# quocdat32461997/ggpm

Measured on AMD Instinct MI355X. Metric: HierMPNEncoder fwd+bwd target row (SURVEY 8(d): encoder + KL heads + optimizer, tree fixed-point hint on; full depth loops in full_depth_loops, the full VAE fwd+bwd row in vae_step) of BASELINE's molecules/sec VAE fwd+bwd (hidden=300, depth=20, batch=32), higher is better.
Workload: dtype f32

## Files before the change

### ggpm_amd/csrc/common.h

```cpp
#pragma once
#include <hip/hip_runtime.h>
#include <stdint.h>
#include <stdlib.h>
#include <atomic>
#include <mutex>
#include "../../include/ggpm_hip.h"

typedef float f32x4 __attribute__((ext_vector_type(4)));
typedef float f32x16 __attribute__((ext_vector_type(16)));

#define GGPM_WAVE 64

#define GGPM_CHECK_LAUNCH()                                   \
    do {                                                      \
        if (hipGetLastError() != hipSuccess) return GGPM_ERR_LAUNCH; \
    } while (0)

#define GGPM_CLEAR_STALE_ERROR() (void)hipGetLastError()

#ifdef GGPM_DEV_SWITCHES
inline const char* ggpm_dev_env(const char* name) { return getenv(name); }
#else
inline const char* ggpm_dev_env(const char*) { return nullptr; }
#endif
// ... 92 lines not shown
    static const ggpm_level_opts none = {};
    return opts ? *opts : none;
}
int ggpm_gru_bias_u_grad(int E1, int H, int depth, int lo, float* work, float* dbu, float* csws, const ggpm_level_opts* opts,
                         ggpm_stream_t stream);
int ggpm_gru_sparse_weight_grads(int E1, int H, int depth, const float* Hs, const float* Ss, const float* Gs, float* work,
                                 size_t work_bytes, float* dWz_h, int ld_dwz, float* dUr, int ld_dur, float* dbu, float* dWh_h,
                                 int ld_dwh, const ggpm_level_opts* opts, ggpm_stream_t stream);
int ggpm_lstm_sparse_weight_grads(int E1, int H, int depth, const float* Hs, const float* Ss, float* work, size_t work_bytes,
                                  float* dWi_h, int ld_dwi, float* dWo_h, int ld_dwo, float* dWu_h, int ld_dwu, float* dWf_h,
                                  int ld_dwf, const ggpm_level_opts* opts, ggpm_stream_t stream);
hipEvent_t ggpm_wgrad_event(int i);

bool ggpm_bf16_storage_applies(int E1, int H);
int ggpm_sum_slots_any(const float* src, int slots, size_t slot_floats, float* out, bool src_bf16, ggpm_stream_t stream);
int ggpm_colsum_any(const float* A, int lda, int rows, int cols, float* out, float* scratch, bool a_bf16, ggpm_stream_t stream);

void ggpm_timing_tag(int tag);
void ggpm_timing_begin(int which, hipStream_t s, double flops);
void ggpm_timing_end(int which, hipStream_t s);
```

### ggpm_amd/csrc/encoder.hip

```cpp
#include "common.h"
#include <condition_variable>
#include <cstring>
#include <cstdlib>
#include <deque>
#include <functional>
#include <mutex>
#include <thread>

hipEvent_t ggpm_wgrad_event(int i);

namespace {

struct Arena {
    char* base;
    size_t off;
    bool overflow;
    size_t cap;
    template <typename T>
    T* take(size_t n) {
        const size_t bytes = (n * sizeof(T) + 255) & ~(size_t)255;
        T* p = base ? reinterpret_cast<T*>(base + off) : nullptr;
        off += bytes;
        if (base && off > cap) overflow = true;
        return p;
// ... 271 lines not shown

inline bool bf16_stored(const Dims& d, int E1) { return d.gate_dtype == 1 && ggpm_bf16_storage_applies(E1, d.H); }
inline int run_steps(const Dims& d, int level, int depth, int E1) {
    static const bool off = ggpm_dev_env("GGPM_TREE_FIXED_POINT") && atoi(ggpm_dev_env("GGPM_TREE_FIXED_POINT")) == 0;
    if (off || level == 2 || bf16_stored(d, E1) || d.tree_chain <= 0 || d.tree_chain + 1 >= depth) return depth;
    return d.tree_chain + 1;
}

inline int backward_lo(const Dims& d, int level, int depth, int E1) {
    static const bool off = ggpm_dev_env("GGPM_TREE_FIXED_POINT") && atoi(ggpm_dev_env("GGPM_TREE_FIXED_POINT")) == 0;
    if (off || level == 2 || bf16_stored(d, E1) || d.tree_chain <= 0) return 1;
    const int lo = depth - d.tree_chain + 1;
    return lo < 1 ? 1 : lo;
}

int replicate_tail(const Dims& d, int E1, int depth, int run, int level, const LevelSaved& L, ggpm_stream_t s) {
    if (run >= depth) return GGPM_OK;
    const size_t slot = (size_t)E1 * d.Hp, ds = (size_t)depth * slot;
    const int blo = backward_lo(d, level, depth, E1);
    ReplicateArgs r = {};
    int n = 0;
    auto add = [&](float* base, int src, int lo, int hi) {
        r.base[n] = base; r.src[n] = src; r.lo[n] = lo > src ? lo : src + 1; r.hi[n] = hi; ++n;
    };
    add(L.Hs, run, blo, depth);
    if (L.Cs) add(L.Cs, run, blo, depth);
    add(L.Qs, run, blo, depth - 1);
    for (int k = 0; k < 5; ++k) add(L.St + k * ds, run - 1, blo - 1, depth - 1);
    r.slot4 = slot / 4;
    dim3 grid((unsigned)ggpm_ceil_div((int)r.slot4, 256 * 4), n);
    replicate_slots_k<<<grid, 256, 0, (hipStream_t)s>>>(r);
    return GGPM_OK;
}

int level_forward(const Dims& d, int E1, int N1, int I, int depth, const float* x, int ldx, float* const* P, int level,
                  const Csr& pred, const Csr& agr, LevelSaved& L, ggpm_stream_t s) {
    const int H = d.H, Hp = d.Hp;
    const size_t slot = (size_t)E1 * Hp;
    const int run = run_steps(d, level, depth, E1);
    struct Tag { Tag(int level) { ggpm_timing_tag(3 - level); } ~Tag() { ggpm_timing_tag(0); } } tag(level);
    ggpm_level_opts o = level_opts(d);
    o.run_depth = run;
    const bool infer = L.hout != nullptr;
    o.h_out = L.hout;
    const float* result = infer ? L.hout : L.Hs + (size_t)depth * slot;
    if (d.lstm) {
        const float* W[4] = {P[lq(level, Q_WI)], P[lq(level, Q_WOG)], P[lq(level, Q_WU)], P[lq(level, Q_WF)]};
        const float* b[4] = {P[lq(level, Q_BI)], P[lq(level, Q_BOG)], P[lq(level, Q_BU)], P[lq(level, Q_BF)]};
        GgpmGemmProblem gp[4];
        for (int k = 0; k < 4; ++k) gp[k] = {x, ldx, W[k], I + H, L.X + k * slot, Hp, Hp, b[k], 0, GGPM_ACT_NONE, 0};
        CK(ggpm_gemm_grouped(0, 1, E1, H, I, 4, gp, s));
        const size_t dsl = (size_t)depth * slot;
        CK(ggpm_lstm_forward(E1, H, depth, L.X, L.X + slot, L.X + 2 * slot, L.X + 3 * slot, W[0] + I, I + H, W[1] + I, I + H,
                             W[2] + I, I + H, W[3] + I, I + H, pred.rowptr, pred.col, L.Hs, L.Cs, L.Qs,
                             infer ? nullptr : L.St, infer ? nullptr : L.St + dsl, infer ? nullptr : L.St + 2 * dsl,
                             infer ? nullptr : L.St + 3 * dsl, infer ? nullptr : L.St + 4 * dsl, L.wpack, infer ? 0 : 1, &o, s));
        if (!infer) CK(replicate_tail(d, E1, depth, run, level, L, s));
        CK(ggpm_segment_sum(result, Hp, agr.rowptr, agr.col, N1, H, L.nei, Hp, 0, Hp, s));
        return GGPM_OK;
    }
// ... 272 lines not shown
        return GGPM_OK;
    });
}

int level_backward(const Dims& d, int E1, int I, int depth, const float* x, int ldx, float* const* P, float* const* G,
                   int level, const Csr& pred, const LevelSaved& L, const float* dHD, float* dX, float* level_work,
                   float* dx, int lddx, BwdWork& w, Streams& st) {
    const int H = d.H, Hp = d.Hp;
    const size_t slot = (size_t)E1 * Hp, ds = (size_t)depth * slot;
    const int blo = backward_lo(d, level, depth, E1);
    struct Tag { Tag(int level) { ggpm_timing_tag(3 - level); } ~Tag() { ggpm_timing_tag(0); } } tag(level);
    static const bool xsum_env = !(ggpm_dev_env("GGPM_SKIP_XSUM") && atoi(ggpm_dev_env("GGPM_SKIP_XSUM")) == 0);
    const bool skip_xsum = xsum_env && dx == nullptr && depth > 1;
    ggpm_level_opts o = level_opts(d);
    o.lo = blo;
    o.skip_x_sums = skip_xsum;
    if (d.lstm) {
        const float* W[4] = {P[lq(level, Q_WI)], P[lq(level, Q_WOG)], P[lq(level, Q_WU)], P[lq(level, Q_WF)]};
        float* dW[4] = {G[lq(level, Q_WI)], G[lq(level, Q_WOG)], G[lq(level, Q_WU)], G[lq(level, Q_WF)]};
        float* db[4] = {G[lq(level, Q_BI)], G[lq(level, Q_BOG)], G[lq(level, Q_BU)], G[lq(level, Q_BF)]};
        CK(ggpm_lstm_backward(E1, H, depth, L.X + 3 * slot, W[0] + I, I + H, W[1] + I, I + H, W[2] + I, I + H, W[3] + I, I + H,
                              pred.rowptr, pred.col, pred.rowptrT, pred.colT, L.Hs, L.Cs, L.Qs, L.St, L.St + ds,
                              L.St + 2 * ds, L.St + 3 * ds, L.St + 4 * ds, dHD, dX, dX + slot, dX + 2 * slot, dX + 3 * slot,
                              dW[0] + I, I + H, dW[1] + I, I + H, dW[2] + I, I + H, dW[3] + I, I + H, level_work,
                              w.level_work_bytes, 0, &o, st.main));
        if (dx) {
            const float* A[4] = {dX, dX + slot, dX + 2 * slot, dX + 3 * slot};
            const int lda[4] = {Hp, Hp, Hp, Hp}, ldb[4] = {I + H, I + H, I + H, I + H}, K[4] = {H, H, H, H};
            CK(ggpm_gemm_ksegments(0, E1, I, 4, A, lda, W, ldb, K, dx, lddx, lddx, nullptr, 0, GGPM_ACT_NONE, 0, st.main));
        }
// ... 254 lines not shown
```

### ggpm_amd/csrc/gemm.hip

```cpp
#include <stdio.h>
#include <stdlib.h>
#include "common.h"

namespace {

constexpr int BM = 64, BN = 64, BK = 32, LDT = 68;

struct GemmArgs {
    int M, N, K;
    const float* A; int lda;
    const float* B; int ldb;
    float* C; int ldc; int n_pad;
    const float* bias;
    int accumulate, act, zero_row0;
    int vecA, vecB;
    int k_chunk;
    float* ws;
    unsigned long long* dbg;
    int nseg;
    const float* segA[GGPM_GEMM_MAX_GROUP];
    const float* segB[GGPM_GEMM_MAX_GROUP];
    int seg_lda[GGPM_GEMM_MAX_GROUP], seg_ldb[GGPM_GEMM_MAX_GROUP], segK[GGPM_GEMM_MAX_GROUP];
};

// ... 1203 lines not shown
        gg.p[i].k_chunk = ggpm_round_up(ggpm_ceil_div(K[i], splits), (bf16 || split) ? BTK : TK);
        gg.p[i].ws = ws + (size_t)i * splits * slabs_per_chunk * (slab / sizeof(float));
    }
    for (int i = count; i < GGPM_GEMM_MAX_GROUP; ++i) gg.p[i] = gg.p[0];
    hipStream_t s = (hipStream_t)stream;
    const int tiles_n = ggpm_ceil_div(N, TN), tiles_m = ggpm_ceil_div(M, TM);
    if (in16) gemm_tn_tall_bf16<true><<<dim3(tiles_n, tiles_m, splits * count), 256, 0, s>>>(gg, splits);
    else if (bf16) gemm_tn_tall_bf16<false><<<dim3(tiles_n, tiles_m, splits * count), 256, 0, s>>>(gg, splits);
    else if (split) launch_tall_split(gg, dim3(tiles_n, tiles_m, splits * count), splits, s);
    else gemm_tn_tall<<<dim3(tiles_n, tiles_m, splits * count), 256, 0, s>>>(gg, splits);
    tall_reduce<<<dim3(tiles_n * tiles_m * 100, count), 256, 0, s>>>(gg, splits * slabs_per_chunk, tiles_n, tiles_n * tiles_m);
    GGPM_CHECK_LAUNCH();
    return GGPM_OK;
}

bool ggpm_bf16_storage_applies(int E1, int H) {
    static const int use_tall = [] { const char* e = ggpm_dev_env("GGPM_GEMM_TALL"); return e ? atoi(e) : 1; }();
    return use_tall && E1 >= 6144 && tall_shape(H, H, E1);
}
extern "C" int ggpm_level_bf16_storage(int E1, int H) { return ggpm_bf16_storage_applies(E1, H) ? 1 : 0; }

extern "C" int ggpm_gemm_tn_bf16_applies(int M, int N, int K) {
    static const int use_tall = [] { const char* e = ggpm_dev_env("GGPM_GEMM_TALL"); return e ? atoi(e) : 1; }();
    return use_tall && M > 0 && N > 0 && K > 0 && tall_shape(M, N, K) ? 1 : 0;
}

extern "C" int ggpm_gemm_tn_bf16(int M, int N, int K, const float* A, int lda, const float* B, int ldb, float* C, int ldc,
                                 float* ws, size_t ws_bytes, ggpm_stream_t stream) {
    if (!A || !B || !C || !ws || M <= 0 || N <= 0 || K <= 0 || ldc < N) return GGPM_ERR_ARG;
    const GgpmGemmProblem p = {A, lda, B, ldb, C, ldc, N, nullptr, 0, GGPM_ACT_NONE, 0};
// ... 184 lines not shown
```

### ggpm_amd/csrc/mpn_gru.hip

```cpp
#include "tile_mma.h"
#include <cstdlib>
#include <cstdio>

__global__ void ggpm_pack_weight_kernel(GgpmPackArgs a) {
    const int Hp = a.Hp, H = a.H, KC = Hp / 16;
    const int lane = threadIdx.x;
    const int kc = blockIdx.x, t = blockIdx.y, m = blockIdx.z;
    const float* __restrict__ W = a.W[m];
    const int ldw = a.ldw[m];
    const int out = 16 * t + (lane & 15);
    if (a.bf16 == 2) {
        const int KC32 = ggpm_kc32_dev(Hp);
        float x[8];
#pragma unroll
        for (int i = 0; i < 8; ++i) {
            const int k = 32 * kc + 8 * (lane >> 4) + i;
            x[i] = (out < H && k < H) ? (a.transpose ? W[(size_t)k * ldw + out] : W[(size_t)out * ldw + k]) : 0.f;
        }
        uint2 lo[3], hi[3];
        ggpm_split3(make_float4(x[0], x[1], x[2], x[3]), lo[0], lo[1], lo[2]);
        ggpm_split3(make_float4(x[4], x[5], x[6], x[7]), hi[0], hi[1], hi[2]);
        __bf16* dst = reinterpret_cast<__bf16*>(a.dst) + (size_t)m * 2 * ggpm_packed_matrix_floats(Hp, 2);
#pragma unroll
        for (int pl = 0; pl < 3; ++pl)
// ... 857 lines not shown
        if (gathered) { a0.src_h = o.gather_h; a0.src_idx = o.gather_idx; }
        const size_t lds_b = bf16 == 2 ? ggpm_split_image_bytes(ROWS, Hp) : (size_t)ROWS * (Hp + 4) * sizeof(float);
        dim3 grid_a(ggpm_ceil_div(E1, ROWS), ggpm_ceil_div(Hp / 16, tg0));
        if (bf16 == 2) { set_lds(gru_fwd_b<2, 1>, lds_b); gru_fwd_b<2, 1><<<grid_a, GGPM_NWA * 64, lds_b, s>>>(a0); }
        else if (bf16 == 1) { set_lds(gru_fwd_b<1, 1>, lds_b); gru_fwd_b<1, 1><<<grid_a, GGPM_NWA * 64, lds_b, s>>>(a0); }
        else { set_lds(gru_fwd_b<0, 1>, lds_b); gru_fwd_b<0, 1><<<grid_a, GGPM_NWA * 64, lds_b, s>>>(a0); }
    }

    const int tg = pick_tg(E1, Hp / 16);
    const double flops1 = 2.0 * (double)(E1 - 1) * H * H;
    static const char* const abl = ggpm_dev_env("GGPM_ABLATE");
    const bool infer = !save_for_backward && o.h_out;
    const bool st16 = bf16 == 1 && !frozen && (save_for_backward || infer) && ggpm_bf16_storage_applies(E1, H);
    int run_depth = o.run_depth;
    if (run_depth <= 0 || run_depth > depth || frozen || !(save_for_backward || infer)) run_depth = depth;
    for (int t = 1; t <= run_depth; ++t) {
        GruFwdArgs a = {};
        a.E1 = E1; a.Hp = Hp; a.tg = tg; a.Xz = Xz; a.Xr = Xr; a.Xh = Xh;
        a.Wz = pWz; a.Wh = pWh; a.Ur = pUr; a.bu = pbu; a.rowptr = pred_rowptr; a.col = pred_col;
        a.ablate = abl ? atoi(abl) : 0;
        a.frozen = frozen;
        a.bf16 = bf16;
        a.st16 = st16 ? 1 : 0;
        a.h0_zero = (t == 1 && !frozen) ? 1 : 0;
        if (save_for_backward) {
            a.Hprev = ggpm_slot_ptr(Hs, t - 1, slot, st16); a.Hnew = ggpm_slot_ptr(Hs, t, slot, st16);
            a.Hout = (st16 && t == depth) ? Hs + (size_t)depth * slot : nullptr;
            a.Qprev = ggpm_slot_ptr(Qs, t - 1, slot, st16);
            a.Qnew = (t < depth) ? ggpm_slot_ptr(Qs, t, slot, st16) : nullptr;
            a.S = ggpm_slot_ptr(Ss, t - 1, slot, st16); a.G = ggpm_slot_ptr(Gs, t - 1, slot, st16);
            a.Z = ggpm_slot_ptr(Zs, t - 1, slot, st16); a.M = ggpm_slot_ptr(Ms, t - 1, slot, st16);
            a.R = Rs + (size_t)(t - 1) * slot;
        } else if (infer) {
            a.Hprev = ggpm_slot_ptr(Hs, (t - 1) & 1, slot, st16); a.Hnew = ggpm_slot_ptr(Hs, t & 1, slot, st16);
            a.Qprev = ggpm_slot_ptr(Qs, (t - 1) & 1, slot, st16); a.Qnew = ggpm_slot_ptr(Qs, t & 1, slot, st16);
            if (t == run_depth) {
                if (st16) a.Hout = o.h_out;
                else a.Hnew = o.h_out;
            }
            a.S = a.G = a.Z = a.M = a.R = nullptr;
        } else {
            a.Hprev = Hs + (size_t)((t - 1) & 1) * slot; a.Hnew = Hs + (size_t)(t & 1) * slot;
            a.Qprev = Qs + (size_t)((t - 1) & 1) * slot; a.Qnew = Qs + (size_t)(t & 1) * slot;
            a.S = a.G = a.Z = a.M = a.R = nullptr;
        }
        launch_fwd(a, rt2, save_for_backward != 0, t < depth, flops1, s);
    }
    GGPM_CHECK_LAUNCH();
    return GGPM_OK;
}

extern "C" int ggpm_gru_forward(int E1, int H, int depth, const float* Xz, const float* Xr, const float* Xh,
                                const float* Wz_h, int ld_wz, const float* Ur, int ld_ur, const float* bu,
                                const float* Wh_h, int ld_wh, const int32_t* pred_rowptr,
                                const int32_t* pred_col, float* Hs, float* Qs, float* Ss, float* Gs, float* Zs,
                                float* Ms, float* Rs, float* wpack, int save_for_backward,
                                const ggpm_level_opts* opts, ggpm_stream_t stream) {
    return gru_forward_impl(E1, H, depth, Xz, Xr, Xh, Wz_h, ld_wz, Ur, ld_ur, bu, Wh_h, ld_wh, pred_rowptr, pred_col,
                            Hs, Qs, Ss, Gs, Zs, Ms, Rs, wpack, save_for_backward, nullptr, nullptr, ggpm_opts_or_default(opts),
                            stream);
}
// ... 82 lines not shown
    }

    {
        GgpmPackArgs pk = {};
        pk.W[0] = Wz_h; pk.ldw[0] = ld_wz; pk.W[1] = Wh_h; pk.ldw[1] = ld_wh; pk.W[2] = Ur; pk.ldw[2] = ld_ur;
        pk.H = H; pk.Hp = Hp; pk.transpose = 1; pk.dst = pWzT; pk.bias = nullptr; pk.bias_out = nullptr; pk.bf16 = bf16;
        if (!o.weights_packed) ggpm_launch_pack(pk, 3, s);
    }
    if (depth == 1 && !frozen) (void)hipMemsetAsync(dXr, 0, slot * sizeof(float), s);

    const int tg = pick_tg(E1, Hp / 16);
    const double flops1 = 2.0 * (double)(E1 - 1) * H * H;
    const bool st16 = bf16 == 1 && !frozen && ggpm_bf16_storage_applies(E1, H);
    int lo = o.lo;
    if (lo < 1 || lo > depth || frozen) lo = 1;
    for (int t = depth; t >= lo; --t) {
        GruBwdArgs a = {};
        a.E1 = E1; a.Hp = Hp; a.tg = tg; a.first = (t == depth);
        a.Xr = Xr;
        a.st16 = st16 ? 1 : 0;
        a.Hcur = ggpm_slot_ptr(Hs, t, slot, st16);
        a.Qcur = (t < depth) ? ggpm_slot_ptr(Qs, t, slot, st16) : nullptr;
        a.S = ggpm_slot_ptr(Ss, t - 1, slot, st16); a.Z = ggpm_slot_ptr(Zs, t - 1, slot, st16);
        a.M = ggpm_slot_ptr(Ms, t - 1, slot, st16);
        a.R = Rs + (size_t)(t - 1) * slot;
        a.dHD = dHD;
        a.dSin = dSb[(t + 1) & 1]; a.dGin = dGb[(t + 1) & 1];
        a.dSout = dSb[t & 1]; a.dGout = dGb[t & 1];
        a.DQ = (t < depth) ? ggpm_slot_ptr(DQ, t, slot, st16) : nullptr;
        a.frozen = frozen; a.carry = carry; a.final_pass = 0; a.dHin = nullptr;
        a.DMP = ggpm_slot_ptr(DMP, t - 1, slot, st16); a.DZP = ggpm_slot_ptr(DZP, t - 1, slot, st16); a.DSD = DSD;
        a.dXz = dXz; a.dXr = dXr; a.dXh = dXh;
        a.WzT = pWzT; a.WhT = pWhT; a.UrT = pUrT; a.bf16 = bf16;
        a.srowptr = succ_rowptr; a.scol = succ_col;
        a.skip_xsum = skip_xsum ? 1 : 0;
        launch_bwd(a, rt2, t > 1 || frozen != nullptr, flops1, s);
    }
    GGPM_CHECK_LAUNCH();

    if (frozen) {
// ... 55 lines not shown
    const int Hp = ggpm_padded_hidden(H);
    hipStream_t s = (hipStream_t)stream;
    const size_t HH = (size_t)Hp * Hp, slot = (size_t)E1 * Hp;
    float* w = work + 3 * ggpm_packed_matrix_slot(Hp);
    float* DMP = w; w += (size_t)depth * slot;
    float* DZP = w; w += (size_t)depth * slot;
    float* DQ = w; w += (size_t)depth * slot;
    w += 6 * slot;
    float* csws = w; w += (size_t)256 * Hp;
    float* skws = w;
    const size_t skbytes = work_bytes - (size_t)((char*)skws - (char*)work);
    const int KD = (depth - lo + 1) * E1;
    const bool st16 = o.gate_dtype == 1 && !with_slot0 && ggpm_bf16_storage_applies(E1, H);
    const int tall_mode = st16 ? 2 : (o.gate_dtype == 1 ? 1 : 0);
    int rc;
    ggpm_gemm_problem gp[3] = {{ggpm_slot_ptr(DMP, lo - 1, slot, st16), Hp, ggpm_slot_ptr(Gs, lo - 1, slot, st16), Hp, dWh_h, ld_dwh, H,
                                nullptr, 0, GGPM_ACT_NONE, 0},
                               {ggpm_slot_ptr(DZP, lo - 1, slot, st16), Hp, ggpm_slot_ptr(Ss, lo - 1, slot, st16), Hp, dWz_h, ld_dwz, H,
                                nullptr, 0, GGPM_ACT_NONE, 0},
                               {nullptr, Hp, nullptr, Hp, dUr, ld_dur, H, nullptr, 0, GGPM_ACT_NONE, 0}};
    int Ks[3] = {KD, KD, 0};
    if (depth > lo || with_slot0) {
        const int first_slot = with_slot0 ? 0 : lo;
        const int KQ = (depth - first_slot) * E1;
        const float* dq0 = ggpm_slot_ptr(DQ, first_slot, slot, st16);
        gp[2].A = dq0;
        gp[2].B = ggpm_slot_ptr(Hs, first_slot, slot, st16);
        Ks[2] = KQ;
        if (!skip_bu) {
            rc = ggpm_colsum_any(dq0, Hp, KQ, H, dbu, csws, st16, stream);
// ... 24 lines not shown
        return GGPM_OK;
    }
    const bool st16 = ggpm_opts_or_default(opts).gate_dtype == 1 && ggpm_bf16_storage_applies(E1, H);
    return ggpm_colsum_any(ggpm_slot_ptr(DQ, lo, slot, st16), Hp, (depth - lo) * E1, H, dbu, csws, st16, stream);
}

namespace {
template <bool B16>
__global__ void __launch_bounds__(256) sum_slots_k(const float* __restrict__ src, int slots, size_t slot4, float* __restrict__ out) {
    const size_t i = (size_t)blockIdx.x * 256 + threadIdx.x;
    if (i >= slot4) return;
    float4 acc = ggpm_ldx<B16>(src, 4 * i);
    for (int t = 1; t < slots; ++t) acc = acc + ggpm_ldx<B16>(src, 4 * ((size_t)t * slot4 + i));
    reinterpret_cast<float4*>(out)[i] = acc;
}
}

extern "C" int ggpm_sum_slots(const float* src, int slots, size_t slot_floats, float* out, ggpm_stream_t stream) {
    return ggpm_sum_slots_any(src, slots, slot_floats, out, false, stream);
}

int ggpm_sum_slots_any(const float* src, int slots, size_t slot_floats, float* out, bool src_bf16, ggpm_stream_t stream) {
    GGPM_CLEAR_STALE_ERROR();
    if (!src || !out || slots <= 0 || slot_floats == 0 || (slot_floats & 3)) return GGPM_ERR_ARG;
    const size_t slot4 = slot_floats / 4;
    if (src_bf16) sum_slots_k<true><<<(unsigned)((slot4 + 255) / 256), 256, 0, (hipStream_t)stream>>>(src, slots, slot4, out);
    else sum_slots_k<false><<<(unsigned)((slot4 + 255) / 256), 256, 0, (hipStream_t)stream>>>(src, slots, slot4, out);
    GGPM_CHECK_LAUNCH();
    return GGPM_OK;
}
// ... 55 lines not shown
```

### ggpm_amd/csrc/mpn_lstm.hip

```cpp
#include "tile_mma.h"
#include <cstdlib>

namespace {

constexpr int ROWS = 16;

struct LstmFwdArgs {
    int E1, Hp, tg;
    const float *Xi, *Xo, *Xu, *Xf;
    const float *Hprev, *Cprev, *Qprev;
    float *Hnew, *Cnew, *Qnew;
    float *S, *I, *O, *U, *F;
    const float *Wi, *Wo, *Wu, *Wf;
    const int32_t *rowptr, *col;
    const unsigned char* frozen;
    int fuse_b;
    int h0_zero;
    int bf16;
    int st16;
    float* Hout;
    const float *src_h, *src_c;
    const int32_t* src_idx;
};

// ... 744 lines not shown
        dim3 grid_a(ggpm_ceil_div(E1, ROWS), ggpm_ceil_div(Hp / 16, tg));
        if (bf16 == 2) { set_lds(lstm_fwd_b<2, 1>, lb); lstm_fwd_b<2, 1><<<grid_a, GGPM_NWA * 64, lb, s>>>(a0); }
        else if (bf16 == 1) { set_lds(lstm_fwd_b<1, 1>, lb); lstm_fwd_b<1, 1><<<grid_a, GGPM_NWA * 64, lb, s>>>(a0); }
        else { set_lds(lstm_fwd_b<0, 1>, lb); lstm_fwd_b<0, 1><<<grid_a, GGPM_NWA * 64, lb, s>>>(a0); }
    } else {
        (void)hipMemsetAsync(Hs, 0, slot * sizeof(float), s);
        (void)hipMemsetAsync(Cs, 0, slot * sizeof(float), s);
        (void)hipMemsetAsync(Qs, 0, slot * sizeof(float), s);
    }

    const double flops1 = 2.0 * (double)(E1 - 1) * H * H;
    const bool infer = !save_for_backward && o.h_out;
    int run_depth = o.run_depth;
    if (run_depth <= 0 || run_depth > depth || frozen || !(save_for_backward || infer)) run_depth = depth;
    const bool st16 = bf16 == 1 && !frozen && (save_for_backward || infer) && ggpm_bf16_storage_applies(E1, H);
    for (int t = 1; t <= run_depth; ++t) {
        LstmFwdArgs a = {};
        a.E1 = E1; a.Hp = Hp; a.tg = tg; a.Xi = Xi; a.Xo = Xo; a.Xu = Xu; a.Xf = Xf;
        a.Wi = pWi; a.Wo = pWo; a.Wu = pWu; a.Wf = pWf; a.rowptr = pred_rowptr; a.col = pred_col;
        a.frozen = frozen;
        a.bf16 = bf16;
        a.st16 = st16 ? 1 : 0;
        a.h0_zero = (t == 1 && !frozen) ? 1 : 0;
        if (save_for_backward) {
            a.Hprev = ggpm_slot_ptr(Hs, t - 1, slot, st16); a.Hnew = ggpm_slot_ptr(Hs, t, slot, st16);
            a.Hout = (st16 && t == depth) ? Hs + (size_t)depth * slot : nullptr;
            a.Cprev = Cs + (size_t)(t - 1) * slot; a.Cnew = Cs + (size_t)t * slot;
            a.Qprev = ggpm_slot_ptr(Qs, t - 1, slot, st16); a.Qnew = (t < depth) ? ggpm_slot_ptr(Qs, t, slot, st16) : nullptr;
            a.S = ggpm_slot_ptr(Ss, t - 1, slot, st16); a.I = ggpm_slot_ptr(Is, t - 1, slot, st16);
            a.O = ggpm_slot_ptr(Os, t - 1, slot, st16); a.U = ggpm_slot_ptr(Us, t - 1, slot, st16);
            a.F = Fs + (size_t)(t - 1) * slot;
        } else if (infer) {
            a.Hprev = ggpm_slot_ptr(Hs, (t - 1) & 1, slot, st16); a.Hnew = ggpm_slot_ptr(Hs, t & 1, slot, st16);
            a.Cprev = Cs + (size_t)((t - 1) & 1) * slot; a.Cnew = Cs + (size_t)(t & 1) * slot;
            a.Qprev = ggpm_slot_ptr(Qs, (t - 1) & 1, slot, st16); a.Qnew = ggpm_slot_ptr(Qs, t & 1, slot, st16);
            if (t == run_depth) {
                if (st16) a.Hout = o.h_out;
                else a.Hnew = o.h_out;
                if (o.c_out) a.Cnew = o.c_out;
            }
            a.S = a.I = a.O = a.U = a.F = nullptr;
        } else {
            a.Hprev = Hs + (size_t)((t - 1) & 1) * slot; a.Hnew = Hs + (size_t)(t & 1) * slot;
            a.Cprev = Cs + (size_t)((t - 1) & 1) * slot; a.Cnew = Cs + (size_t)(t & 1) * slot;
            a.Qprev = Qs + (size_t)((t - 1) & 1) * slot; a.Qnew = Qs + (size_t)(t & 1) * slot;
            a.S = a.I = a.O = a.U = a.F = nullptr;
        }
        launch_fwd(a, rt2, save_for_backward != 0, t < depth, flops1, s);
    }
    GGPM_CHECK_LAUNCH();
    return GGPM_OK;
}

extern "C" int ggpm_lstm_forward(int E1, int H, int depth, const float* Xi, const float* Xo, const float* Xu,
                                 const float* Xf, const float* Wi_h, int ld_wi, const float* Wo_h, int ld_wo,
                                 const float* Wu_h, int ld_wu, const float* Wf_h, int ld_wf,
                                 const int32_t* pred_rowptr, const int32_t* pred_col, float* Hs, float* Cs,
                                 float* Qs, float* Ss, float* Is, float* Os, float* Us, float* Fs,
                                 float* wpack, int save_for_backward, const ggpm_level_opts* opts, ggpm_stream_t stream) {
    return lstm_forward_impl(E1, H, depth, Xi, Xo, Xu, Xf, Wi_h, ld_wi, Wo_h, ld_wo, Wu_h, ld_wu, Wf_h, ld_wf, pred_rowptr,
                             pred_col, Hs, Cs, Qs, Ss, Is, Os, Us, Fs, wpack, save_for_backward, nullptr, nullptr,
                             nullptr, ggpm_opts_or_default(opts), stream);
}
// ... 79 lines not shown
    (void)skws; (void)skbytes;

    {
        GgpmPackArgs pk = {};
        pk.W[0] = Wi_h; pk.ldw[0] = ld_wi; pk.W[1] = Wo_h; pk.ldw[1] = ld_wo; pk.W[2] = Wu_h; pk.ldw[2] = ld_wu;
        pk.W[3] = Wf_h; pk.ldw[3] = ld_wf;
        pk.H = H; pk.Hp = Hp; pk.transpose = 1; pk.dst = pWiT; pk.bias = nullptr; pk.bias_out = nullptr; pk.bf16 = bf16;
        if (!o.weights_packed) ggpm_launch_pack(pk, 4, s);
    }

    const int tg = pick_tg(E1, Hp / 16);
    const double flops1 = 2.0 * (double)(E1 - 1) * H * H;
    int lo = o.lo;
    if (lo < 1 || lo > depth || frozen) lo = 1;
    const bool st16 = bf16 == 1 && !frozen && ggpm_bf16_storage_applies(E1, H);
    for (int t = depth; t >= lo; --t) {
        LstmBwdArgs a = {};
        a.E1 = E1; a.Hp = Hp; a.tg = tg; a.first = (t == depth);
        a.st16 = st16 ? 1 : 0;
        a.Xf = Xf;
        a.Ccur = Cs + (size_t)t * slot;
        a.Qcur = (t < depth) ? ggpm_slot_ptr(Qs, t, slot, st16) : nullptr;
        a.F = Fs + (size_t)(t - 1) * slot;
        a.I = ggpm_slot_ptr(Is, t - 1, slot, st16); a.O = ggpm_slot_ptr(Os, t - 1, slot, st16);
        a.U = ggpm_slot_ptr(Us, t - 1, slot, st16);
        a.dHD = dHD;
        a.dSin = dSb[(t + 1) & 1]; a.dFCin = dFb[(t + 1) & 1];
        a.dSout = dSb[t & 1]; a.dFCout = dFb[t & 1];
        a.DQ = (t < depth) ? ggpm_slot_ptr(DQ, t, slot, st16) : nullptr;
        a.frozen = frozen; a.dCD = dCD; a.carry_h = carry_h; a.carry_c = carry_c; a.final_pass = 0;
        a.dHin = nullptr; a.dCin = nullptr;
        a.DI = ggpm_slot_ptr(DI, t - 1, slot, st16); a.DO = ggpm_slot_ptr(DO, t - 1, slot, st16);
        a.DU = ggpm_slot_ptr(DU, t - 1, slot, st16);
        a.dXi = dXi; a.dXo = dXo; a.dXu = dXu; a.dXf = dXf;
        a.WiT = pWiT; a.WoT = pWoT; a.WuT = pWuT; a.WfT = pWfT; a.bf16 = bf16;
        a.srowptr = succ_rowptr; a.scol = succ_col;
        a.skip_xsum = skip_xsum ? 1 : 0;
        launch_bwd(a, rt2, t > 1 || frozen != nullptr, flops1, s);
    }
    GGPM_CHECK_LAUNCH();
// ... 69 lines not shown
    hipStream_t s = (hipStream_t)stream;
    const size_t HH = (size_t)Hp * Hp, slot = (size_t)E1 * Hp;
    float* w = work + 4 * ggpm_packed_matrix_slot(Hp);
    float* DI = w; w += (size_t)depth * slot;
    float* DO = w; w += (size_t)depth * slot;
    float* DU = w; w += (size_t)depth * slot;
    float* DQ = w; w += (size_t)depth * slot;
    w += 6 * slot;
    float* skws = w;
    const size_t skbytes = work_bytes - (size_t)((char*)skws - (char*)work);
    const int KD = (depth - lo + 1) * E1;
    const bool st16 = o.gate_dtype == 1 && !with_slot0 && ggpm_bf16_storage_applies(E1, H);
    const int tall_mode = st16 ? 2 : (o.gate_dtype == 1 ? 1 : 0);
    const float* Sl = ggpm_slot_ptr(Ss, lo - 1, slot, st16);
    int rc;
    ggpm_gemm_problem gp[4] = {{ggpm_slot_ptr(DI, lo - 1, slot, st16), Hp, Sl, Hp, dWi_h, ld_dwi, H, nullptr, 0, GGPM_ACT_NONE, 0},
                               {ggpm_slot_ptr(DO, lo - 1, slot, st16), Hp, Sl, Hp, dWo_h, ld_dwo, H, nullptr, 0, GGPM_ACT_NONE, 0},
                               {ggpm_slot_ptr(DU, lo - 1, slot, st16), Hp, Sl, Hp, dWu_h, ld_dwu, H, nullptr, 0, GGPM_ACT_NONE, 0},
                               {nullptr, Hp, nullptr, Hp, dWf_h, ld_dwf, H, nullptr, 0, GGPM_ACT_NONE, 0}};
    int Ks[4] = {KD, KD, KD, 0};
    if (depth > lo || with_slot0) {
        const int first_slot = with_slot0 ? 0 : lo;
        gp[3].A = ggpm_slot_ptr(DQ, first_slot, slot, st16);
        gp[3].B = ggpm_slot_ptr(Hs, first_slot, slot, st16);
        Ks[3] = (depth - first_slot) * E1;
        rc = ggpm_gemm_tall_grouped(H, H, 4, gp, Ks, skws, skbytes, stream, tall_mode);
        if (rc) return rc;
    } else {
        rc = ggpm_gemm_tall_grouped(H, H, 3, gp, Ks, skws, skbytes, stream, tall_mode);
        if (rc) return rc;
// ... 46 lines not shown
```

### ggpm_amd/functional.py

```python
from __future__ import annotations

import ctypes
import os
import weakref
from typing import List, Optional, Sequence, Tuple

import torch

from . import _dev, _lib
from .nnutils import version_of
from .parallel import grad_view

ACT_NONE, ACT_RELU, ACT_TANH, ACT_SIGMOID = 0, 1, 2, 3


def _stream() -> ctypes.c_void_p:
    return ctypes.c_void_p(torch._C._cuda_getCurrentRawStream(torch._C._cuda_getDevice()))


def _p(t: Optional[torch.Tensor]) -> ctypes.c_void_p:
    return ctypes.c_void_p(0 if t is None else t.data_ptr())


def _need_gpu(*ts: torch.Tensor) -> None:
# ... 184 lines not shown
                ("K", ctypes.c_int)]


class GemmProblem(ctypes.Structure):
    _fields_ = [("A", ctypes.c_void_p), ("lda", ctypes.c_int), ("B", ctypes.c_void_p), ("ldb", ctypes.c_int),
                ("C", ctypes.c_void_p), ("ldc", ctypes.c_int), ("n_pad", ctypes.c_int), ("bias", ctypes.c_void_p),
                ("accumulate", ctypes.c_int), ("act", ctypes.c_int), ("zero_row0", ctypes.c_int)]


class LevelOpts(ctypes.Structure):
    _fields_ = [("gate_dtype", ctypes.c_int), ("prefer_narrow", ctypes.c_int), ("weights_packed", ctypes.c_int),
                ("defer_stash", ctypes.c_void_p * 4), ("gather_h", ctypes.c_void_p), ("gather_c", ctypes.c_void_p),
                ("gather_idx", ctypes.c_void_p), ("scatter_h", ctypes.c_void_p), ("scatter_c", ctypes.c_void_p),
                ("scatter_idx", ctypes.c_void_p), ("skip_x_sums", ctypes.c_int), ("run_depth", ctypes.c_int),
                ("lo", ctypes.c_int), ("skip_bias_u", ctypes.c_int), ("skip_sparse_wgrads", ctypes.c_int),
                ("h_out", ctypes.c_void_p), ("c_out", ctypes.c_void_p)]


_GATE_OPTS = {dt: LevelOpts(gate_dtype=dt) for dt in (1, 2, 3)}


def _gate_opts(gate_dtype: int):
    o = _GATE_OPTS.get(gate_dtype)
    return None if o is None else ctypes.byref(o)


def gemm_grouped(ta: int, tb: int, M: int, N: int, K: int, problems, splitk: bool = False) -> None:
    lib = _lib.load()
    arr = _lib.array_type(GemmProblem, len(problems))()
    for i, q in enumerate(problems):
        arr[i] = GemmProblem(_p(q["A"]), q["lda"], _p(q["B"]), q["ldb"], _p(q["C"]), q["ldc"], q["n_pad"],
# ... 918 lines not shown
```

### include/ggpm_hip.h

```cpp
#ifndef GGPM_HIP_H
#define GGPM_HIP_H

#include <stddef.h>
#include <stdint.h>

#ifdef __cplusplus
extern "C" {
#endif

typedef void* ggpm_stream_t;

enum {
    GGPM_OK = 0,
    GGPM_ERR_ARG = 1,
    GGPM_ERR_LAUNCH = 2,
    GGPM_ERR_UNSUPPORTED = 3,
    GGPM_ERR_WORKSPACE = 4
};

enum { GGPM_ACT_NONE = 0, GGPM_ACT_RELU = 1, GGPM_ACT_TANH = 2, GGPM_ACT_SIGMOID = 3 };

int ggpm_version(void);
const char* ggpm_error_string(int code);
int ggpm_padded_hidden(int H);
// ... 96 lines not shown
    int weights_packed;
    float* defer_stash[4];
    const float* gather_h;
    const float* gather_c;
    const int32_t* gather_idx;
    float* scatter_h;
    float* scatter_c;
    const int32_t* scatter_idx;
    int skip_x_sums;
    int run_depth;
    int lo;
    int skip_bias_u;
    int skip_sparse_wgrads;
    float* h_out;
    float* c_out;
} ggpm_level_opts;

size_t ggpm_gru_pack_floats(int H);
int ggpm_gru_forward(int E1, int H, int depth, const float* Xz, const float* Xr, const float* Xh,
                     const float* Wz_h, int ld_wz, const float* Ur, int ld_ur, const float* bu,
                     const float* Wh_h, int ld_wh, const int32_t* pred_rowptr, const int32_t* pred_col,
                     float* Hs, float* Qs, float* Ss, float* Gs, float* Zs, float* Ms, float* Rs,
                     float* wpack, int save_for_backward, const ggpm_level_opts* opts, ggpm_stream_t stream);
size_t ggpm_gru_backward_workspace_bytes(int E1, int H, int depth);
int ggpm_gru_backward(int E1, int H, int depth, const float* Xr, const float* Wz_h, int ld_wz,
                      const float* Ur, int ld_ur, const float* Wh_h, int ld_wh,
                      const int32_t* pred_rowptr, const int32_t* pred_col, const int32_t* succ_rowptr,
                      const int32_t* succ_col, const float* Hs, const float* Qs, const float* Ss,
                      const float* Gs, const float* Zs, const float* Ms, const float* Rs, const float* dHD, float* dXz,
                      float* dXr, float* dXh, float* dWz_h, int ld_dwz, float* dUr, int ld_dur,
// ... 233 lines not shown
```

Measured before the change: 11840.

## Use single fixed stash slot for converged tree depth, skip tail replication

When the tree fixed-point hint says the recurrence converges at run depth before full depth, the forward pass stashes gate activations only at that step. The backward pass reuses that single slot for all later steps instead of replicating tail slots. Weight gradients are computed by summing the per-step gate gradients into compensated hi/lo pairs (two-sum) and running one grouped TN GEMM against the fixed stashed state. This removes the tail replication copies, the per-step stash writes and the multi-slot tall GEMMs, at the cost of a new summation kernel and a two-segment GEMM.

```diff
diff --git a/ggpm_amd/csrc/common.h b/ggpm_amd/csrc/common.h
--- a/ggpm_amd/csrc/common.h
+++ b/ggpm_amd/csrc/common.h
@@ -130,6 +130,10 @@
 
 bool ggpm_bf16_storage_applies(int E1, int H);
 int ggpm_sum_slots_any(const float* src, int slots, size_t slot_floats, float* out, bool src_bf16, ggpm_stream_t stream);
+int ggpm_sum_slots_pair_grouped(int count, const float* const* src, const int* slots, size_t slot_floats, float* const* hi,
+                                float* const* lo, ggpm_stream_t stream);
+struct ggpm_pair_problem { const float *hi, *lo, *B; float* C; int ldc; };
+int ggpm_gemm_tn_pair_grouped(int M, int N, int rows, int ld, int count, const ggpm_pair_problem* p, ggpm_stream_t stream);
 int ggpm_colsum_any(const float* A, int lda, int rows, int cols, float* out, float* scratch, bool a_bf16, ggpm_stream_t stream);
 
 void ggpm_timing_tag(int tag);
diff --git a/ggpm_amd/csrc/encoder.hip b/ggpm_amd/csrc/encoder.hip
--- a/ggpm_amd/csrc/encoder.hip
+++ b/ggpm_amd/csrc/encoder.hip
@@ -309,8 +309,15 @@
     return lo < 1 ? 1 : lo;
 }
 
+inline int fixed_slot(const Dims& d, int level, int depth, int E1) {
+    const int run = run_steps(d, level, depth, E1);
+    if (run >= depth || d.gate_dtype == 1) return 0;
+    const int blo = backward_lo(d, level, depth, E1);
+    return (blo >= run && blo >= 3) ? run : 0;
+}
+
 int replicate_tail(const Dims& d, int E1, int depth, int run, int level, const LevelSaved& L, ggpm_stream_t s) {
-    if (run >= depth) return GGPM_OK;
+    if (run >= depth || fixed_slot(d, level, depth, E1)) return GGPM_OK;
     const size_t slot = (size_t)E1 * d.Hp, ds = (size_t)depth * slot;
     const int blo = backward_lo(d, level, depth, E1);
     ReplicateArgs r = {};
@@ -338,7 +345,9 @@
     o.run_depth = run;
     const bool infer = L.hout != nullptr;
     o.h_out = L.hout;
-    const float* result = infer ? L.hout : L.Hs + (size_t)depth * slot;
+    const int fs = infer ? 0 : fixed_slot(d, level, depth, E1);
+    o.fixed_slot = fs;
+    const float* result = infer ? L.hout : L.Hs + (size_t)(fs ? fs : depth) * slot;
     if (d.lstm) {
         const float* W[4] = {P[lq(level, Q_WI)], P[lq(level, Q_WOG)], P[lq(level, Q_WU)], P[lq(level, Q_WF)]};
         const float* b[4] = {P[lq(level, Q_BI)], P[lq(level, Q_BOG)], P[lq(level, Q_BU)], P[lq(level, Q_BF)]};
@@ -641,6 +650,7 @@
     const bool skip_xsum = xsum_env && dx == nullptr && depth > 1;
     ggpm_level_opts o = level_opts(d);
     o.lo = blo;
+    o.fixed_slot = fixed_slot(d, level, depth, E1);
     o.skip_x_sums = skip_xsum;
     if (d.lstm) {
         const float* W[4] = {P[lq(level, Q_WI)], P[lq(level, Q_WOG)], P[lq(level, Q_WU)], P[lq(level, Q_WF)]};
diff --git a/ggpm_amd/csrc/gemm.hip b/ggpm_amd/csrc/gemm.hip
--- a/ggpm_amd/csrc/gemm.hip
+++ b/ggpm_amd/csrc/gemm.hip
@@ -1241,6 +1241,40 @@
     return GGPM_OK;
 }
 
+int ggpm_gemm_tn_pair_grouped(int M, int N, int rows, int ld, int count, const ggpm_pair_problem* p, ggpm_stream_t stream) {
+    GGPM_CLEAR_STALE_ERROR();
+    if (count <= 0 || count > GGPM_GEMM_MAX_GROUP || !p || M <= 0 || N <= 0 || rows <= 0 || ld < M || ld < N) return GGPM_ERR_ARG;
+    bool ok = small_launch(M, N, count);
+    for (int i = 0; i < count; ++i) {
+        if (!p[i].hi || !p[i].lo || !p[i].B || !p[i].C || p[i].ldc < N) return GGPM_ERR_ARG;
+        ok = ok && v2_operands_ok(p[i].hi, ld, rows, p[i].B, ld, rows) && v2_operands_ok(p[i].lo, ld, rows, p[i].B, ld, rows);
+    }
+    if (!ok) {
+        for (int i = 0; i < count; ++i) {
+            int rc = ggpm_gemm(1, 0, M, N, rows, p[i].hi, ld, p[i].B, ld, p[i].C, p[i].ldc, N, nullptr, 0, GGPM_ACT_NONE, 0,
+                               nullptr, 0, stream);
+            if (rc) return rc;
+            rc = ggpm_gemm(1, 0, M, N, rows, p[i].lo, ld, p[i].B, ld, p[i].C, p[i].ldc, N, nullptr, 1, GGPM_ACT_NONE, 0,
+                           nullptr, 0, stream);
+            if (rc) return rc;
+        }
+        return GGPM_OK;
+    }
+    GemmGroupArgs gg;
+    for (int i = 0; i < count; ++i) {
+        const GgpmGemmProblem q = {p[i].hi, ld, p[i].B, ld, p[i].C, p[i].ldc, N, nullptr, 0, GGPM_ACT_NONE, 0};
+        GemmArgs& g = gg.p[i];
+        fill_args(g, M, N, rows, q);
+        g.nseg = 2;
+        g.segA[0] = p[i].hi; g.segA[1] = p[i].lo;
+        for (int sg = 0; sg < 2; ++sg) { g.segB[sg] = p[i].B; g.seg_lda[sg] = g.seg_ldb[sg] = ld; g.segK[sg] = rows; }
+    }
+    for (int i = count; i < GGPM_GEMM_MAX_GROUP; ++i) gg.p[i] = gg.p[0];
+    launch_small(1, 0, gg, count, M, N, (hipStream_t)stream);
+    GGPM_CHECK_LAUNCH();
+    return GGPM_OK;
+}
+
 bool ggpm_bf16_storage_applies(int E1, int H) {
     static const int use_tall = [] { const char* e = ggpm_dev_env("GGPM_GEMM_TALL"); return e ? atoi(e) : 1; }();
     return use_tall && E1 >= 6144 && tall_shape(H, H, E1);
diff --git a/ggpm_amd/csrc/mpn_gru.hip b/ggpm_amd/csrc/mpn_gru.hip
--- a/ggpm_amd/csrc/mpn_gru.hip
+++ b/ggpm_amd/csrc/mpn_gru.hip
@@ -895,7 +895,10 @@
     const bool st16 = bf16 == 1 && !frozen && (save_for_backward || infer) && ggpm_bf16_storage_applies(E1, H);
     int run_depth = o.run_depth;
     if (run_depth <= 0 || run_depth > depth || frozen || !(save_for_backward || infer)) run_depth = depth;
+    const int fs = (o.fixed_slot > 0 && save_for_backward && !frozen && !st16) ? o.fixed_slot : 0;
+    if (fs && fs != run_depth) return GGPM_ERR_ARG;
     for (int t = 1; t <= run_depth; ++t) {
+        const bool stash = save_for_backward && (!fs || t == fs);
         GruFwdArgs a = {};
         a.E1 = E1; a.Hp = Hp; a.tg = tg; a.Xz = Xz; a.Xr = Xr; a.Xh = Xh;
         a.Wz = pWz; a.Wh = pWh; a.Ur = pUr; a.bu = pbu; a.rowptr = pred_rowptr; a.col = pred_col;
@@ -912,6 +915,7 @@
             a.S = ggpm_slot_ptr(Ss, t - 1, slot, st16); a.G = ggpm_slot_ptr(Gs, t - 1, slot, st16);
             a.Z = ggpm_slot_ptr(Zs, t - 1, slot, st16); a.M = ggpm_slot_ptr(Ms, t - 1, slot, st16);
             a.R = Rs + (size_t)(t - 1) * slot;
+            if (!stash) a.S = a.G = a.Z = a.M = a.R = nullptr;
         } else if (infer) {
             a.Hprev = ggpm_slot_ptr(Hs, (t - 1) & 1, slot, st16); a.Hnew = ggpm_slot_ptr(Hs, t & 1, slot, st16);
             a.Qprev = ggpm_slot_ptr(Qs, (t - 1) & 1, slot, st16); a.Qnew = ggpm_slot_ptr(Qs, t & 1, slot, st16);
@@ -925,7 +929,7 @@
             a.Qprev = Qs + (size_t)((t - 1) & 1) * slot; a.Qnew = Qs + (size_t)(t & 1) * slot;
             a.S = a.G = a.Z = a.M = a.R = nullptr;
         }
-        launch_fwd(a, rt2, save_for_backward != 0, t < depth, flops1, s);
+        launch_fwd(a, rt2, stash, t < depth, flops1, s);
     }
     GGPM_CHECK_LAUNCH();
     return GGPM_OK;
@@ -1038,16 +1042,20 @@
     const bool st16 = bf16 == 1 && !frozen && ggpm_bf16_storage_applies(E1, H);
     int lo = o.lo;
     if (lo < 1 || lo > depth || frozen) lo = 1;
+    const int fs = (o.fixed_slot > 0 && !frozen && !st16) ? o.fixed_slot : 0;
+    if (fs && (fs >= depth || lo < fs)) return GGPM_ERR_ARG;
+    auto state_slot = [fs](int t) { return fs && t > fs ? fs : t; };
+    auto stash_slot = [fs](int t) { return fs && t > fs ? fs - 1 : t - 1; };
     for (int t = depth; t >= lo; --t) {
         GruBwdArgs a = {};
         a.E1 = E1; a.Hp = Hp; a.tg = tg; a.first = (t == depth);
         a.Xr = Xr;
         a.st16 = st16 ? 1 : 0;
-        a.Hcur = ggpm_slot_ptr(Hs, t, slot, st16);
-        a.Qcur = (t < depth) ? ggpm_slot_ptr(Qs, t, slot, st16) : nullptr;
-        a.S = ggpm_slot_ptr(Ss, t - 1, slot, st16); a.Z = ggpm_slot_ptr(Zs, t - 1, slot, st16);
-        a.M = ggpm_slot_ptr(Ms, t - 1, slot, st16);
-        a.R = Rs + (size_t)(t - 1) * slot;
+        a.Hcur = ggpm_slot_ptr(Hs, state_slot(t), slot, st16);
+        a.Qcur = (t < depth) ? ggpm_slot_ptr(Qs, state_slot(t), slot, st16) : nullptr;
+        a.S = ggpm_slot_ptr(Ss, stash_slot(t), slot, st16); a.Z = ggpm_slot_ptr(Zs, stash_slot(t), slot, st16);
+        a.M = ggpm_slot_ptr(Ms, stash_slot(t), slot, st16);
+        a.R = Rs + (size_t)stash_slot(t) * slot;
         a.dHD = dHD;
         a.dSin = dSb[(t + 1) & 1]; a.dGin = dGb[(t + 1) & 1];
         a.dSout = dSb[t & 1]; a.dGout = dGb[t & 1];
@@ -1133,6 +1141,33 @@
     const bool st16 = o.gate_dtype == 1 && !with_slot0 && ggpm_bf16_storage_applies(E1, H);
     const int tall_mode = st16 ? 2 : (o.gate_dtype == 1 ? 1 : 0);
     int rc;
+    if (o.fixed_slot > 0 && !with_slot0) {
+        const int fs = o.fixed_slot;
+        if (fs >= depth || lo < fs || lo < 3 || o.gate_dtype == 1) return GGPM_ERR_ARG;
+        const int nq = depth - lo;
+        const float* src[3] = {DMP + (size_t)(lo - 1) * slot, DZP + (size_t)(lo - 1) * slot, DQ + (size_t)lo * slot};
+        const int slots[3] = {depth - lo + 1, depth - lo + 1, nq};
+        float* const hi[3] = {DMP, DZP, DQ};
+        float* const lw[3] = {DMP + slot, DZP + slot, DQ + slot};
+        rc = ggpm_sum_slots_pair_grouped(nq > 0 ? 3 : 2, src, slots, slot, hi, lw, stream);
+        if (rc) return rc;
+        const ggpm_pair_problem pp[3] = {{DMP, DMP + slot, Gs + (size_t)(fs - 1) * slot, dWh_h, ld_dwh},
+                                         {DZP, DZP + slot, Ss + (size_t)(fs - 1) * slot, dWz_h, ld_dwz},
+                                         {DQ, DQ + slot, Hs + (size_t)fs * slot, dUr, ld_dur}};
+        if (nq > 0) {
+            if (!skip_bu) {
+                rc = ggpm_colsum(DQ, Hp, 2 * E1, H, dbu, csws, stream);
+                if (rc) return rc;
+            }
+        } else {
+            for (int r = 0; r < H; ++r) (void)hipMemsetAsync(dUr + (size_t)r * ld_dur, 0, H * sizeof(float), s);
+            if (!skip_bu) (void)hipMemsetAsync(dbu, 0, H * sizeof(float), s);
+        }
+        rc = ggpm_gemm_tn_pair_grouped(H, H, E1, Hp, nq > 0 ? 3 : 2, pp, stream);
+        if (rc) return rc;
+        GGPM_CHECK_LAUNCH();
+        return GGPM_OK;
+    }
     ggpm_gemm_problem gp[3] = {{ggpm_slot_ptr(DMP, lo - 1, slot, st16), Hp, ggpm_slot_ptr(Gs, lo - 1, slot, st16), Hp, dWh_h, ld_dwh, H,
                                 nullptr, 0, GGPM_ACT_NONE, 0},
                                {ggpm_slot_ptr(DZP, lo - 1, slot, st16), Hp, ggpm_slot_ptr(Ss, lo - 1, slot, st16), Hp, dWz_h, ld_dwz, H,
@@ -1187,6 +1222,49 @@
     for (int t = 1; t < slots; ++t) acc = acc + ggpm_ldx<B16>(src, 4 * ((size_t)t * slot4 + i));
     reinterpret_cast<float4*>(out)[i] = acc;
 }
+}
+
+namespace {
+struct SumPairArgs {
+    const float* src[4];
+    float *hi[4], *lo[4];
+    int slots[4];
+    size_t slot4;
+};
+__device__ __forceinline__ void two_sum(float a, float b, float& s, float& e) {
+    s = a + b;
+    const float bb = s - a;
+    e = (a - (s - bb)) + (b - bb);
+}
+__global__ void __launch_bounds__(256) sum_slots_pair_k(SumPairArgs p) {
+    const int m = blockIdx.y;
+    const size_t i = (size_t)blockIdx.x * 256 + threadIdx.x;
+    if (i >= p.slot4) return;
+    const float4* __restrict__ src = reinterpret_cast<const float4*>(p.src[m]);
+    float4 h = src[i], l = ggpm_zero4(), e;
+    for (int t = 1; t < p.slots[m]; ++t) {
+        const float4 x = src[(size_t)t * p.slot4 + i];
+        two_sum(h.x, x.x, h.x, e.x); two_sum(h.y, x.y, h.y, e.y); two_sum(h.z, x.z, h.z, e.z); two_sum(h.w, x.w, h.w, e.w);
+        l = l + e;
+    }
+    reinterpret_cast<float4*>(p.hi[m])[i] = h;
+    reinterpret_cast<float4*>(p.lo[m])[i] = l;
+}
+}
+
+int ggpm_sum_slots_pair_grouped(int count, const float* const* src, const int* slots, size_t slot_floats, float* const* hi,
+                                float* const* lo, ggpm_stream_t stream) {
+    GGPM_CLEAR_STALE_ERROR();
+    if (count <= 0 || count > 4 || !src || !slots || !hi || !lo || slot_floats == 0 || (slot_floats & 3)) return GGPM_ERR_ARG;
+    SumPairArgs p = {};
+    for (int m = 0; m < count; ++m) {
+        if (!src[m] || !hi[m] || !lo[m] || slots[m] <= 0) return GGPM_ERR_ARG;
+        p.src[m] = src[m]; p.hi[m] = hi[m]; p.lo[m] = lo[m]; p.slots[m] = slots[m];
+    }
+    p.slot4 = slot_floats / 4;
+    sum_slots_pair_k<<<dim3((unsigned)((p.slot4 + 255) / 256), count), 256, 0, (hipStream_t)stream>>>(p);
+    GGPM_CHECK_LAUNCH();
+    return GGPM_OK;
 }
 
 extern "C" int ggpm_sum_slots(const float* src, int slots, size_t slot_floats, float* out, ggpm_stream_t stream) {
diff --git a/ggpm_amd/csrc/mpn_lstm.hip b/ggpm_amd/csrc/mpn_lstm.hip
--- a/ggpm_amd/csrc/mpn_lstm.hip
+++ b/ggpm_amd/csrc/mpn_lstm.hip
@@ -782,7 +782,10 @@
     int run_depth = o.run_depth;
     if (run_depth <= 0 || run_depth > depth || frozen || !(save_for_backward || infer)) run_depth = depth;
     const bool st16 = bf16 == 1 && !frozen && (save_for_backward || infer) && ggpm_bf16_storage_applies(E1, H);
+    const int fs = (o.fixed_slot > 0 && save_for_backward && !frozen && !st16) ? o.fixed_slot : 0;
+    if (fs && fs != run_depth) return GGPM_ERR_ARG;
     for (int t = 1; t <= run_depth; ++t) {
+        const bool stash = save_for_backward && (!fs || t == fs);
         LstmFwdArgs a = {};
         a.E1 = E1; a.Hp = Hp; a.tg = tg; a.Xi = Xi; a.Xo = Xo; a.Xu = Xu; a.Xf = Xf;
         a.Wi = pWi; a.Wo = pWo; a.Wu = pWu; a.Wf = pWf; a.rowptr = pred_rowptr; a.col = pred_col;
@@ -798,6 +801,7 @@
             a.S = ggpm_slot_ptr(Ss, t - 1, slot, st16); a.I = ggpm_slot_ptr(Is, t - 1, slot, st16);
             a.O = ggpm_slot_ptr(Os, t - 1, slot, st16); a.U = ggpm_slot_ptr(Us, t - 1, slot, st16);
             a.F = Fs + (size_t)(t - 1) * slot;
+            if (!stash) a.S = a.I = a.O = a.U = a.F = nullptr;
         } else if (infer) {
             a.Hprev = ggpm_slot_ptr(Hs, (t - 1) & 1, slot, st16); a.Hnew = ggpm_slot_ptr(Hs, t & 1, slot, st16);
             a.Cprev = Cs + (size_t)((t - 1) & 1) * slot; a.Cnew = Cs + (size_t)(t & 1) * slot;
@@ -814,7 +818,7 @@
             a.Qprev = Qs + (size_t)((t - 1) & 1) * slot; a.Qnew = Qs + (size_t)(t & 1) * slot;
             a.S = a.I = a.O = a.U = a.F = nullptr;
         }
-        launch_fwd(a, rt2, save_for_backward != 0, t < depth, flops1, s);
+        launch_fwd(a, rt2, stash, t < depth, flops1, s);
     }
     GGPM_CHECK_LAUNCH();
     return GGPM_OK;
@@ -924,16 +928,20 @@
     int lo = o.lo;
     if (lo < 1 || lo > depth || frozen) lo = 1;
     const bool st16 = bf16 == 1 && !frozen && ggpm_bf16_storage_applies(E1, H);
+    const int fs = (o.fixed_slot > 0 && !frozen && !st16) ? o.fixed_slot : 0;
+    if (fs && (fs >= depth || lo < fs)) return GGPM_ERR_ARG;
+    auto state_slot = [fs](int t) { return fs && t > fs ? fs : t; };
+    auto stash_slot = [fs](int t) { return fs && t > fs ? fs - 1 : t - 1; };
     for (int t = depth; t >= lo; --t) {
         LstmBwdArgs a = {};
         a.E1 = E1; a.Hp = Hp; a.tg = tg; a.first = (t == depth);
         a.st16 = st16 ? 1 : 0;
         a.Xf = Xf;
-        a.Ccur = Cs + (size_t)t * slot;
-        a.Qcur = (t < depth) ? ggpm_slot_ptr(Qs, t, slot, st16) : nullptr;
-        a.F = Fs + (size_t)(t - 1) * slot;
-        a.I = ggpm_slot_ptr(Is, t - 1, slot, st16); a.O = ggpm_slot_ptr(Os, t - 1, slot, st16);
-        a.U = ggpm_slot_ptr(Us, t - 1, slot, st16);
+        a.Ccur = Cs + (size_t)state_slot(t) * slot;
+        a.Qcur = (t < depth) ? ggpm_slot_ptr(Qs, state_slot(t), slot, st16) : nullptr;
+        a.F = Fs + (size_t)stash_slot(t) * slot;
+        a.I = ggpm_slot_ptr(Is, stash_slot(t), slot, st16); a.O = ggpm_slot_ptr(Os, stash_slot(t), slot, st16);
+        a.U = ggpm_slot_ptr(Us, stash_slot(t), slot, st16);
         a.dHD = dHD;
         a.dSin = dSb[(t + 1) & 1]; a.dFCin = dFb[(t + 1) & 1];
         a.dSout = dSb[t & 1]; a.dFCout = dFb[t & 1];
@@ -1033,6 +1041,27 @@
     const int tall_mode = st16 ? 2 : (o.gate_dtype == 1 ? 1 : 0);
     const float* Sl = ggpm_slot_ptr(Ss, lo - 1, slot, st16);
     int rc;
+    if (o.fixed_slot > 0 && !with_slot0) {
+        const int fs = o.fixed_slot;
+        if (fs >= depth || lo < fs || lo < 3 || o.gate_dtype == 1) return GGPM_ERR_ARG;
+        const int nq = depth - lo;
+        const float* src[4] = {DI + (size_t)(lo - 1) * slot, DO + (size_t)(lo - 1) * slot, DU + (size_t)(lo - 1) * slot,
+                               DQ + (size_t)lo * slot};
+        const int slots[4] = {depth - lo + 1, depth - lo + 1, depth - lo + 1, nq};
+        float* const hi[4] = {DI, DO, DU, DQ};
+        float* const lw[4] = {DI + slot, DO + slot, DU + slot, DQ + slot};
+        rc = ggpm_sum_slots_pair_grouped(nq > 0 ? 4 : 3, src, slots, slot, hi, lw, stream);
+        if (rc) return rc;
+        const float* Sf = Ss + (size_t)(fs - 1) * slot;
+        const ggpm_pair_problem pp[4] = {{DI, DI + slot, Sf, dWi_h, ld_dwi}, {DO, DO + slot, Sf, dWo_h, ld_dwo},
+                                         {DU, DU + slot, Sf, dWu_h, ld_dwu}, {DQ, DQ + slot, Hs + (size_t)fs * slot, dWf_h, ld_dwf}};
+        if (nq == 0)
+            for (int r = 0; r < H; ++r) (void)hipMemsetAsync(dWf_h + (size_t)r * ld_dwf, 0, H * sizeof(float), s);
+        rc = ggpm_gemm_tn_pair_grouped(H, H, E1, Hp, nq > 0 ? 4 : 3, pp, stream);
+        if (rc) return rc;
+        GGPM_CHECK_LAUNCH();
+        return GGPM_OK;
+    }
     ggpm_gemm_problem gp[4] = {{ggpm_slot_ptr(DI, lo - 1, slot, st16), Hp, Sl, Hp, dWi_h, ld_dwi, H, nullptr, 0, GGPM_ACT_NONE, 0},
                                {ggpm_slot_ptr(DO, lo - 1, slot, st16), Hp, Sl, Hp, dWo_h, ld_dwo, H, nullptr, 0, GGPM_ACT_NONE, 0},
                                {ggpm_slot_ptr(DU, lo - 1, slot, st16), Hp, Sl, Hp, dWu_h, ld_dwu, H, nullptr, 0, GGPM_ACT_NONE, 0},
diff --git a/ggpm_amd/functional.py b/ggpm_amd/functional.py
--- a/ggpm_amd/functional.py
+++ b/ggpm_amd/functional.py
@@ -222,7 +222,7 @@
                 ("gather_idx", ctypes.c_void_p), ("scatter_h", ctypes.c_void_p), ("scatter_c", ctypes.c_void_p),
                 ("scatter_idx", ctypes.c_void_p), ("skip_x_sums", ctypes.c_int), ("run_depth", ctypes.c_int),
                 ("lo", ctypes.c_int), ("skip_bias_u", ctypes.c_int), ("skip_sparse_wgrads", ctypes.c_int),
-                ("h_out", ctypes.c_void_p), ("c_out", ctypes.c_void_p)]
+                ("h_out", ctypes.c_void_p), ("c_out", ctypes.c_void_p), ("fixed_slot", ctypes.c_int)]
 
 
 _GATE_OPTS = {dt: LevelOpts(gate_dtype=dt) for dt in (1, 2, 3)}
diff --git a/include/ggpm_hip.h b/include/ggpm_hip.h
--- a/include/ggpm_hip.h
+++ b/include/ggpm_hip.h
@@ -134,6 +134,7 @@
     int skip_sparse_wgrads;
     float* h_out;
     float* c_out;
+    int fixed_slot;
 } ggpm_level_opts;
 
 size_t ggpm_gru_pack_floats(int H);
```

Result: faster. 12190, median of 6 (+3.0%).
